# MisEty/GPS-SLAM

Measured on AMD Instinct MI355X. Metric: SLAM frames/sec @640x480, ~200k Gaussians; render PSNR vs ref, higher is better.
Workload: dtype f32; 1 GPU; synthetic RGB-D SLAM frames, independent scene per GPU; env_overrides=, full=False, schedule=overlap, windows=1, local_opt_interval=10, local_opt_iters=20, use_gt_pose=False, prologue_frames=25

## Files before the change

### gps_slam_amd/_lib.py

```python
import ctypes as C
import os

_HERE = os.path.dirname(os.path.abspath(__file__))
_LIBPATH = os.path.join(_HERE, "libgpsslam_hip.so")
_lib = None

vp, i32, i64, f32, f64 = C.c_void_p, C.c_int, C.c_int64, C.c_float, C.c_double


class TsdfState(C.Structure):
    _fields_ = [("width", i32), ("height", i32), ("fx", f32), ("fy", f32), ("cx", f32), ("cy", f32),
                ("voxel_size", f32), ("mu", f32), ("view_frustum_min", f32), ("view_frustum_max", f32),
                ("max_w", i32), ("n_blocks", i32), ("n_buckets", i32), ("n_excess", i32),
                ("vba", vp), ("vba_alloc_list", vp), ("hash", vp), ("excess_list", vp), ("counters", vp),
                ("alloc_prio", vp), ("scan_scratch", vp), ("visible_type", vp), ("visible_ids", vp), ("depth", vp),
                ("rgb", vp), ("minmax", vp), ("raycast", vp), ("icp_points", vp), ("icp_normals", vp),
                ("fv_visible_ids", vp), ("fv_minmax", vp), ("fv_raycast", vp), ("fv_colour", vp)]


class TsdfView(C.Structure):
    _fields_ = [("M", f32 * 16), ("invM", f32 * 16), ("fx", f32), ("fy", f32), ("cx", f32), ("cy", f32),
                ("visible_ids", vp), ("minmax", vp), ("raycast", vp), ("colour", vp), ("scratch", vp), ("counters", vp),
                ("w2c", f32 * 16), ("color_map", vp), ("vertex_map", vp), ("confidence_map", vp), ("depth_map", vp),
                ("depth_map_clamped", vp)]
# ... 52 lines not shown
    "gps_ssim_bwd": (i32, [i32, i32, i32, i32, i32, vp, vp, vp, vp, vp, vp, vp, vp]),
    "gps_upload_floats": (i32, [vp, vp, i32, vp]),
    "gps_isect_tiles": (i32, [i32, vp, vp, vp, i32, i32, i32, i64, vp, vp, vp, vp, vp, vp, i64, vp]),
    "gps_raster_raw_fwd": (i32, [i32, vp, vp, vp, vp, vp, i32, i32, i32, vp, vp, vp, vp, vp, vp, vp]),
    "gps_raster_raw_bwd": (i32, [i32, vp, vp, vp, vp, vp, i32, i32, i32, vp, vp, vp, vp, vp, vp, vp, vp, vp, vp, vp, vp,
                                 vp]),
    "gps_raster_ges_fwd": (i32, [i32, vp, vp, vp, vp, vp, i32, i32, i32, vp, vp, vp, f32, vp, vp, vp, vp]),
    "gps_raster_ges_bwd_gs": (i32, [i32, vp, vp, vp, vp, vp, vp, i32, i32, vp, vp, vp, f32, vp, vp, vp, vp, vp, vp,
                                    i32, vp]),
    "gps_raster_ges_bwd_strips": (i32, [i32, vp, vp, vp, vp, i32, vp, vp, i32, i32, vp, vp]),
    "gps_set_frame_chain_reserve": (None, [i32]),
    "gps_set_raster_fwd_persistent": (None, [i32]),

    "gps_raster_pack_records": (i32, [i32, vp, vp, vp, vp, vp, vp, vp]),
    "gps_raster_pair_image": (i32, [i32, i32, vp, vp, f32, vp, vp]),
    "gps_raster_ges_bwd_exact": (i32, [i32, vp, vp, vp, vp, vp, i32, i32, i32, vp, vp, vp, f32, vp, vp, vp, vp, vp, vp, vp]),
    "gps_compose_l1": (i32, [i32, i32, vp, vp, vp, vp, vp, vp, vp, vp, vp, vp, vp]),
    "gps_adam_step": (i32, [C.POINTER(AdamSegment), i32, f64, f64, f64, i32, vp]),
    "gps_loss_terms_workspace_floats": (i64, [i32, i32]),
    "gps_loss_terms": (i32, [i32, i32, vp, vp, vp, vp, vp, f32, vp, vp, f32, f32, vp, vp, vp, vp, vp, vp, vp, vp, vp]),
    "gps_loss_terms_exposure_partials": (i64, [i32, i32]),
    "gps_loss_terms_exposure": (i32, [i32, i32, vp, vp, vp, vp, vp, f32, vp, vp, f32, f32, vp, vp, vp, vp, vp, vp, vp, vp, vp, vp,
                                      vp]),
    "gps_exposure_slab_floats": (i64, [i32, i32]),
    "gps_compose_exposure": (i32, [i32, i32, vp, vp, vp, vp, vp, vp, vp, vp]),
    "gps_exposure_fwd": (i32, [i32, vp, vp, vp, vp]),
    "gps_exposure_bwd": (i32, [i32, vp, vp, vp, vp, vp, vp]),
    "gps_exposure_reduce": (i32, [vp, i32, i32, i32, vp, vp]),
    "gps_gauss_preprocess_fwd": (i32, [i32, i32, i32, vp, vp, vp, vp, vp, vp, vp, vp, vp, i32, i32, f32, f32, f32, f32,
                                       i32, vp, vp, vp, vp, vp, vp, vp, vp]),
    "gps_raster_ges_fwd_rec": (i32, [i32, vp, vp, i32, i32, vp, vp, vp, f32, vp, vp, vp]),
    "gps_raster_ges_fwd_rec_ordered": (i32, [i32, vp, vp, i32, i32, vp, vp, vp, f32, vp, vp, vp, vp]),
    "gps_isect_workspace_tile_order": (vp, [vp, i32, i64]),
    "gps_gauss_preprocess_bwd": (i32, [i32, i32, i32, vp, vp, vp, vp, vp, vp, vp, vp, vp, i32, i32, f32, vp, vp, vp, vp,
                                       vp, vp, vp, vp, vp, vp, vp, vp, vp]),
    "gps_gauss_preprocess_bwd_adam": (i32, [i32, i32, i32, vp, vp, vp, vp, vp, vp, vp, vp, vp, i32, i32, f32, vp, vp, vp,
                                            vp, vp, vp, vp, vp, vp, vp, vp, vp, vp, vp, f64, vp, f64, f64, f64, i32, vp]),
    "gps_tsdf_scratch_bytes": (i64, [i32, i32, i32, i32]),
    "gps_tsdf_reset": (i32, [C.POINTER(TsdfState), vp]),
    "gps_tsdf_rebuild_index": (i32, [C.POINTER(TsdfState), vp]),
    "gps_tsdf_mesh_workspace_bytes": (i64, [C.POINTER(TsdfState)]),
    "gps_tsdf_mesh_scene": (i32, [C.POINTER(TsdfState), i64, vp, vp, vp, i64, vp]),
    "gps_track_config_init": (i32, [C.POINTER(TrackConfig), C.c_char_p, i32, i32, f32, f32, f32, f32, i32, i32]),
    "gps_track_state_reset": (i32, [C.POINTER(TrackState)]),
    "gps_track_arg_line_alloc": (i32, [C.POINTER(vp)]),
    "gps_track_arg_line_free": (i32, [vp]),
    "gps_track_scratch_bytes": (i64, [i32, i32]),
    "gps_track_poll_profile": (i32, [vp, i32, i32, vp, vp]),
    "gps_track_poll_phases": (i32, [vp, i32, i32, vp, vp]),
    "gps_tsdf_track_camera": (i32, [C.POINTER(TsdfState), C.POINTER(TrackConfig), C.POINTER(TrackState), vp, i64, vp]),
    "gps_tsdf_process_frame_tracked": (i32, [C.POINTER(TsdfState), vp, C.POINTER(TrackConfig), C.POINTER(TrackState), vp, i64,
                                             vp]),
    "gps_tsdf_process_frame_tracked_gated": (i32, [C.POINTER(TsdfState), vp, C.POINTER(TrackConfig), C.POINTER(TrackState), vp, i64,
                                                   vp, vp, vp]),
    "gps_tsdf_convert_depth": (i32, [C.POINTER(TsdfState), vp, vp]),
    "gps_tsdf_allocate": (i32, [C.POINTER(TsdfState), vp, vp, vp]),
    "gps_tsdf_integrate": (i32, [C.POINTER(TsdfState), vp, vp]),
    "gps_tsdf_expected_depths": (i32, [C.POINTER(TsdfState), vp, i32, vp]),
    "gps_tsdf_expected_depths_partial": (i32, [C.POINTER(TsdfState), vp, i32, vp]),
    "gps_tsdf_raycast": (i32, [C.POINTER(TsdfState), vp, i32, i32, vp]),
    "gps_tsdf_expected_depths_and_raycast": (i32, [C.POINTER(TsdfState), vp, vp, i32, i32, vp]),
    "gps_tsdf_icp_maps": (i32, [C.POINTER(TsdfState), vp, vp]),
    "gps_tsdf_ray_stats": (i32, [C.POINTER(TsdfState), vp]),
    "gps_tsdf_ray_wave_rows": (i32, [C.POINTER(TsdfState), vp, i32, vp]),
    "gps_tsdf_find_visible": (i32, [C.POINTER(TsdfState), vp, vp]),
    "gps_tsdf_render_colour": (i32, [C.POINTER(TsdfState), vp]),
# ... 71 lines not shown
```

### gps_slam_amd/csrc/splat_bin.hpp

```cpp
#pragma once
#include "common.hpp"

namespace gps {

constexpr int BIN_BLOCK = 256;

struct TileBox { uint32_t x0, y0, x1, y1; };

__device__ __forceinline__ TileBox tile_bbox(float mx, float my, int radius_i, int tile_size, int tw, int th) {
    float radius = (float)radius_i;
    float ts = (float)tile_size;
    float tr = radius / ts, tx = mx / ts, ty = my / ts;
    TileBox b;
    float fx0 = floorf(tx - tr), fy0 = floorf(ty - tr), fx1 = ceilf(tx + tr), fy1 = ceilf(ty + tr);
    b.x0 = (uint32_t)fminf(fmaxf(fx0, 0.f), (float)tw);
    b.y0 = (uint32_t)fminf(fmaxf(fy0, 0.f), (float)th);
    b.x1 = (uint32_t)fminf(fmaxf(fx1, 0.f), (float)tw);
    b.y1 = (uint32_t)fminf(fmaxf(fy1, 0.f), (float)th);
    return b;
}

__device__ __forceinline__ void tile_group_count(float mx, float my, int r, int tile_size, int tw, int th, int& tiles, int& groups) {
    TileBox b = tile_bbox(mx, my, r, tile_size, tw, th);
    tiles = (int)((b.y1 - b.y0) * (b.x1 - b.x0));
    float rf = (float)r;
    groups = (int)((4 * rf * rf + 32 - 1) / 32);
}

constexpr int SB_MAX = 512;
constexpr int SB_MAX_TILES = 4096;
constexpr int BWD_CLASSES = GPS_BWD_CLASSES;
constexpr int BWD_BANDS = 16;
constexpr int BWD_KEYS = BWD_CLASSES * BWD_BANDS;
struct SbTables {
    uint32_t* C;
    uint32_t* P;
    uint32_t* tile_total;
    int32_t* cls_count;
    int32_t* cls_prefix;
    int sb_shift;
    int32_t* tile_order;
};
bool map_runs_beside_frame_chain();
int frame_chain_reserve_bits();
bool sb_supported(int N, int tile_width, int tile_height);
int sb_tables_clear(const struct SbTables& t, gps_stream stream);
__host__ __device__ inline int sb_shift_for(int N) {
    int s = 0;
    while ((((int64_t)N + 255) / 256 + ((int64_t)1 << s) - 1) >> s > SB_MAX) s++;
    return s;
}
__host__ __device__ inline int bwd_class(int r) { return r <= 4 ? 0 : r <= 8 ? 1 : r <= 16 ? 2 : r <= 32 ? 3 : 4; }
__host__ __device__ inline int bwd_key(int r, int n_tiles, unsigned y0, int th) {
    const int band = n_tiles > 0 ? (int)(y0 * (unsigned)BWD_BANDS / (unsigned)(th > 0 ? th : 1)) : 0;
    return bwd_class(r) * BWD_BANDS + (band < BWD_BANDS ? band : BWD_BANDS - 1);
}

struct BinCountOut {
    int32_t *tiles_per_gauss, *groups_per_gauss, *blk_tiles, *blk_groups, *blk_vis;
    int tile_size, tw, th;
    SbTables sb;
};

__device__ __forceinline__ void bin_block_sums(const BinCountOut& o, int t, int g, int vis) {
    __shared__ int red[3][BIN_BLOCK / 64];
    int ts = wave_sum_i(t), gs = wave_sum_i(g), vs = wave_sum_i(vis);
    if ((threadIdx.x & 63) == 0) { red[0][threadIdx.x >> 6] = ts; red[1][threadIdx.x >> 6] = gs; red[2][threadIdx.x >> 6] = vs; }
    __syncthreads();
    if (threadIdx.x == 0) {
        int a = 0, b = 0, c = 0;
        for (int w = 0; w < BIN_BLOCK / 64; w++) { a += red[0][w]; b += red[1][w]; c += red[2][w]; }
        o.blk_tiles[blockIdx.x] = a; o.blk_groups[blockIdx.x] = b; o.blk_vis[blockIdx.x] = c;
    }
}
// ... 48 lines not shown
```

### gps_slam_amd/csrc/splat_bin_sb.hip

```cpp
#include <mutex>

#include "launch_timing.hpp"
#include "splat_bin.hpp"

namespace {

using gps::BIN_BLOCK;
using gps::SB_MAX;
using gps::SB_MAX_TILES;
using gps::SbTables;
using gps::TileBox;
using gps::tile_bbox;

constexpr int SCAT_THREADS = 512;
constexpr int SCAT_WAVES = SCAT_THREADS / 64;
constexpr int SCAT_ITEMS = 4;
constexpr int SCAT_CHUNK = SCAT_THREADS * SCAT_ITEMS;

__device__ __forceinline__ int wave_max_i(int v) {
#pragma unroll
    for (int o = 32; o > 0; o >>= 1) v = max(v, __shfl_xor(v, o, 64));
    return v;
}
__device__ __forceinline__ int wave_min_i(int v) {
#pragma unroll
    for (int o = 32; o > 0; o >>= 1) v = min(v, __shfl_xor(v, o, 64));
    return v;
}
__device__ __forceinline__ int wave_excl_scan_i(int v, int& total) {
    const int incl = wave_incl_scan_i(v);
    total = __shfl(incl, 63, 64);
    return incl - v;
}

__global__ __launch_bounds__(256) void sb_scan_kernel(int n_tiles, SbTables t, gps::LaunchStamp stamp) {
    gps::StampScope timed(stamp);
    const int lane = threadIdx.x & 63, wave = threadIdx.x >> 6;
    const int tile = blockIdx.x * 4 + wave;
    static_assert(SB_MAX == 512, "a lane owns 8 consecutive superblocks");
    if (tile < n_tiles) {
        uint4* crow = reinterpret_cast<uint4*>(t.C + (size_t)tile * SB_MAX) + 2 * lane;
        const uint4 a = crow[0], b = crow[1];
        crow[0] = make_uint4(0, 0, 0, 0); crow[1] = make_uint4(0, 0, 0, 0);
        const int s = (int)(a.x + a.y + a.z + a.w + b.x + b.y + b.z + b.w);
        int total;
        uint32_t run = (uint32_t)wave_excl_scan_i(s, total);
        uint4 pa, pb;
        pa.x = run; run += a.x; pa.y = run; run += a.y; pa.z = run; run += a.z; pa.w = run; run += a.w;
        pb.x = run; run += b.x; pb.y = run; run += b.y; pb.z = run; run += b.z; pb.w = run;
        uint4* prow = reinterpret_cast<uint4*>(t.P + (size_t)tile * SB_MAX) + 2 * lane;
        prow[0] = pa; prow[1] = pb;
        if (lane == 0) t.tile_total[tile] = (uint32_t)total;
    }
    const int k = tile - n_tiles;
    if (k >= 0 && k < gps::BWD_KEYS) {
        int4* crow = reinterpret_cast<int4*>(t.cls_count + (size_t)k * SB_MAX) + 2 * lane;
        const int4 a = crow[0], b = crow[1];
        crow[0] = make_int4(0, 0, 0, 0); crow[1] = make_int4(0, 0, 0, 0);
        const int s = a.x + a.y + a.z + a.w + b.x + b.y + b.z + b.w;
        int total;
        int run = wave_excl_scan_i(s, total);
        int4 pa, pb;
        pa.x = run; run += a.x; pa.y = run; run += a.y; pa.z = run; run += a.z; pa.w = run; run += a.w;
        pb.x = run; run += b.x; pb.y = run; run += b.y; pb.z = run; run += b.z; pb.w = run;
        int4* prow = reinterpret_cast<int4*>(t.cls_prefix + (size_t)k * SB_MAX) + 2 * lane;
        prow[0] = pa; prow[1] = pb;
        if (lane == 0) t.cls_prefix[gps::BWD_KEYS * SB_MAX + k] = total;
    }
}

__global__ __launch_bounds__(SCAT_THREADS) void sb_scatter_kernel(
    int N, const float* __restrict__ means2d, const int32_t* __restrict__ radii, const int32_t* __restrict__ tiles_per_gauss,
    int tile_size, int tw, int th, SbTables t, int64_t isect_cap, int32_t* __restrict__ flatten_ids,
    int32_t* __restrict__ tile_offsets, int64_t* __restrict__ counts, int32_t* __restrict__ cls_ids,
    int32_t* __restrict__ cls_counts, int64_t cls_stride, gps::LaunchStamp stamp) {
    gps::StampScope timed(stamp);
    extern __shared__ uint32_t lds[];
    const int n_tiles = tw * th;
    if (blockIdx.x == gridDim.x - 1) {
        __shared__ int hist[64];
        __shared__ int gws[SCAT_WAVES];
        const int tid_ = threadIdx.x, lane_ = tid_ & 63, wave_ = tid_ >> 6;
        if (tid_ < 64) hist[tid_] = 0;
        const int per = (n_tiles + SCAT_THREADS - 1) / SCAT_THREADS;
        const int lo = min(n_tiles, tid_ * per), hi = min(n_tiles, lo + per);
        int sum = 0;
        for (int b = lo; b < hi; b++) sum += (int)t.tile_total[b];
        const int incl = wave_incl_scan_i(sum);
        if (lane_ == 63) gws[wave_] = incl;
        __syncthreads();
        int woff = 0, total = 0;
        for (int w = 0; w < SCAT_WAVES; w++) { const int v = gws[w]; if (w < wave_) woff += v; total += v; }
        int64_t run = woff + incl - sum;
        for (int b = lo; b < hi; b++) {
            const int tt = (int)t.tile_total[b];
            tile_offsets[b] = (int)min(run, isect_cap);
            atomicAdd(&hist[63 - min(63, tt >> 5)], 1);
            run += tt;
        }
        if (tid_ == 0) {
            int64_t ni = total;
            if (ni > isect_cap) { ni = isect_cap; counts[2] = 1; }
            counts[0] = ni; counts[1] = 0;
            int nv = 0;
            for (int k = 0; k < gps::BWD_CLASSES; k++) {
                int nk = 0;
                for (int b = 0; b < gps::BWD_BANDS; b++) nk += t.cls_prefix[gps::BWD_KEYS * SB_MAX + k * gps::BWD_BANDS + b];
                if (cls_counts) cls_counts[k] = nk;
                nv += nk;
            }
            counts[3] = nv;
        }
        __syncthreads();
        if (tid_ < 64) {
            int tot_;
            const int ex = wave_excl_scan_i(hist[tid_], tot_);
            hist[tid_] = ex;
        }
        __syncthreads();
        for (int b = tid_; b < n_tiles; b += SCAT_THREADS) t.tile_order[atomicAdd(&hist[63 - min(63, (int)(t.tile_total[b] >> 5))], 1)] = b;
        return;
    }
    const int sb = blockIdx.x, sb_size = BIN_BLOCK << t.sb_shift;
    uint32_t* base = lds;
    uint16_t* wavecnt = reinterpret_cast<uint16_t*>(lds + n_tiles);
    uint16_t* tot16 = wavecnt + SCAT_WAVES * n_tiles;
    uint32_t* pre = lds + n_tiles + ((SCAT_WAVES + 1) * n_tiles + 1) / 2;
    uint32_t* box = pre + sb_size + 1;
    __shared__ int ws[SCAT_WAVES], wlo[SCAT_WAVES], whi[SCAT_WAVES];
    __shared__ int key_wave[SCAT_WAVES][gps::BWD_KEYS];
    __shared__ int key_run[gps::BWD_KEYS];
    const int tid = threadIdx.x, lane = tid & 63, wave = tid >> 6;
    const int g0 = sb * sb_size;

    if (cls_ids && tid < gps::BWD_KEYS) {
        int start = t.cls_prefix[tid * SB_MAX + sb];
        for (int k = tid - tid % gps::BWD_BANDS; k < tid; k++) start += t.cls_prefix[gps::BWD_KEYS * SB_MAX + k];
        key_run[tid] = start;
        for (int w = 0; w < SCAT_WAVES; w++) key_wave[w][tid] = 0;
    }
    int carry = 0, row_lo = th, row_hi = 0;
    for (int j0 = 0; j0 < sb_size; j0 += SCAT_THREADS) {
        const int j = j0 + tid, g = g0 + j;
        const bool mine_j = j < sb_size;
        int tcount = 0, r = 0;
        uint32_t bx = 0;
        if (mine_j && g < N) {
            tcount = tiles_per_gauss[g];
            r = radii[g];
            if (tcount > 0) {
                const float2 m = *reinterpret_cast<const float2*>(means2d + 2 * (size_t)g);
                const TileBox b = tile_bbox(m.x, m.y, r, tile_size, tw, th);
                bx = b.x0 | (b.y0 << 12) | ((b.x1 - b.x0) << 24);
                row_lo = min(row_lo, (int)b.y0); row_hi = max(row_hi, (int)b.y1);
            }
// ... 12 lines not shown
        }
        __syncthreads();
        int woff = 0, total = 0;
        for (int w = 0; w < SCAT_WAVES; w++) { const int v = ws[w]; if (w < wave) woff += v; total += v; }
        if (mine_j) { pre[j] = (uint32_t)(carry + woff + incl - tcount); box[j] = bx; }
        carry += total;
        if (cls_ids) {
            if (key >= 0) {
                int before = 0;
                for (int w = 0; w < wave; w++) before += key_wave[w][key];
                cls_ids[(key / gps::BWD_BANDS) * cls_stride + key_run[key] + before + rank] = g;
            }
            __syncthreads();
            if (tid < gps::BWD_KEYS) {
                int all = 0;
                for (int w = 0; w < SCAT_WAVES; w++) { all += key_wave[w][tid]; key_wave[w][tid] = 0; }
                key_run[tid] += all;
            }
        }
    }
    const int n_pairs = carry;
    row_lo = wave_min_i(row_lo); row_hi = wave_max_i(row_hi);
    __syncthreads();
    if (lane == 0) { wlo[wave] = row_lo; whi[wave] = row_hi; }
    if (tid == 0) pre[sb_size] = (uint32_t)carry;
    __syncthreads();
    for (int w = 0; w < SCAT_WAVES; w++) { row_lo = min(row_lo, wlo[w]); row_hi = max(row_hi, whi[w]); }
    int t_lo = min(row_lo, row_hi) * tw, t_hi = row_hi * tw;
    if (t_hi < t_lo) t_hi = t_lo;
    const int nt = t_hi - t_lo;
    if (n_pairs == 0) return;

    {
        int before = 0;
        for (int b = tid; b < t_lo; b += SCAT_THREADS) before += (int)t.tile_total[b];
        const int per = (nt + SCAT_THREADS - 1) / SCAT_THREADS;
        const int lo = min(nt, tid * per), hi = min(nt, lo + per);
        int sum = 0;
        for (int b = lo; b < hi; b++) sum += (int)t.tile_total[t_lo + b];
        const int incl = wave_incl_scan_i(sum);
        before = wave_sum_i(before);
        __syncthreads();
        if (lane == 63) ws[wave] = incl;
        if (lane == 0) wlo[wave] = before;
        __syncthreads();
        int woff = 0, total = 0, front = 0;
        for (int w = 0; w < SCAT_WAVES; w++) { const int v = ws[w]; if (w < wave) woff += v; total += v; front += wlo[w]; }
        int run = front + woff + incl - sum;
        for (int b = lo; b < hi; b++) {
            base[b] = (uint32_t)run + t.P[(size_t)(t_lo + b) * SB_MAX + sb];
            run += (int)t.tile_total[t_lo + b];
        }
        (void)total;
    }
    int bits = 1;
    while ((1 << bits) < max(nt, 2)) bits++;
    const unsigned long long lt = lanemask_lt();
    uint16_t* mycnt = wavecnt + wave * n_tiles;
    for (int c0 = 0; c0 < n_pairs; c0 += SCAT_CHUNK) {
        for (int k = tid; k < nt; k += SCAT_THREADS) {
#pragma unroll
            for (int w = 0; w < SCAT_WAVES; w++) wavecnt[w * n_tiles + k] = 0;
        }
        __syncthreads();
        uint32_t tile[SCAT_ITEMS], gid[SCAT_ITEMS], rank[SCAT_ITEMS];
#pragma unroll
        for (int k = 0; k < SCAT_ITEMS; k++) {
            const int p = c0 + wave * (64 * SCAT_ITEMS) + k * 64 + lane;
            const bool valid = p < n_pairs;
            uint32_t d = 0;
            gid[k] = 0;
            if (valid) {
                int lo = 0, hi = sb_size;
                while (hi - lo > 1) { const int mid = (lo + hi) >> 1; if ((int)pre[mid] <= p) lo = mid; else hi = mid; }
                const uint32_t b = box[lo];
                const uint32_t w = b >> 24, q = (uint32_t)(p - (int)pre[lo]);
                d = ((b >> 12) & 0xfffu) * (uint32_t)tw + (b & 0xfffu) + (q / w) * (uint32_t)tw + q % w - (uint32_t)t_lo;
                gid[k] = (uint32_t)(g0 + lo);
            }
            tile[k] = d;
            unsigned long long same = __ballot(valid);
            for (int bb = 0; bb < bits; bb++) {
                const unsigned long long bal = __ballot(valid && ((d >> bb) & 1u));
                same &= ((d >> bb) & 1u) ? bal : ~bal;
            }
            const uint32_t prev = mycnt[d];
// ... 49 lines not shown
    static size_t granted[MAX_DEVICES] = {0};
    int dev = 0;
    if (hipGetDevice(&dev) != hipSuccess || dev < 0 || dev >= MAX_DEVICES) { (void)hipGetLastError(); return false; }
    std::lock_guard<std::mutex> lock(mu);
    if (lds <= granted[dev]) return true;
    if (hipFuncSetAttribute(reinterpret_cast<const void*>(sb_scatter_kernel), hipFuncAttributeMaxDynamicSharedMemorySize, (int)lds) != hipSuccess) {
        (void)hipGetLastError();
        return false;
    }
    granted[dev] = lds;
    return true;
}

size_t sb_tables_bytes() {
    return (size_t)SB_MAX_TILES * SB_MAX * 4 * 2 + (size_t)SB_MAX_TILES * 4 * 2 + (size_t)(SB_MAX + 1) * BWD_KEYS * 4 * 2 + 2048;
}

int sb_tables_clear(const SbTables& t, gps_stream stream) {
    hipStream_t s = (hipStream_t)stream;
    const bool ok = hipMemsetAsync(t.C, 0, (size_t)SB_MAX_TILES * SB_MAX * 4, s) == hipSuccess &&
                    hipMemsetAsync(t.cls_count, 0, (size_t)(SB_MAX + 1) * BWD_KEYS * 4, s) == hipSuccess;
    return ok ? GPS_OK : GPS_ERR_LAUNCH;
}

void sb_tables_carve(char* base, SbTables* t) {
    size_t off = 0;
    auto take = [&](size_t bytes) { char* p = base + off; off += (bytes + 255) & ~(size_t)255; return p; };
    t->C = (uint32_t*)take((size_t)SB_MAX_TILES * SB_MAX * 4);
    t->P = (uint32_t*)take((size_t)SB_MAX_TILES * SB_MAX * 4);
    t->tile_total = (uint32_t*)take((size_t)SB_MAX_TILES * 4);
    t->cls_count = (int32_t*)take((size_t)(SB_MAX + 1) * BWD_KEYS * 4);
    t->cls_prefix = (int32_t*)take((size_t)(SB_MAX + 1) * BWD_KEYS * 4);
    t->tile_order = (int32_t*)take((size_t)SB_MAX_TILES * 4);
    t->sb_shift = 0;
}

int isect_tiles_superblock(int N, const float* means2d, const int32_t* radii, const BinCountOut& cnt, int64_t isect_capacity,
                           const int32_t* tiles_per_gauss, int32_t* flatten_ids, int32_t* tile_offsets, int64_t* counts,
                           int32_t* cls_ids, int32_t* cls_counts, int64_t cls_stride, gps_stream stream) {
    GPS_ENTER();
    const int n_tiles = cnt.tw * cnt.th;
    hipStream_t s = (hipStream_t)stream;
    const bool ok = N > 0 && cnt.sb.C && isect_capacity > 0 && means2d && radii && tiles_per_gauss && flatten_ids && tile_offsets &&
                    counts && (!cls_ids || (cls_counts && cls_stride >= N)) && cnt.sb.sb_shift == sb_shift_for(N) &&
                    sb_supported(N, cnt.tw, cnt.th);
    if (!ok) {
        if (cnt.sb.C) (void)sb_tables_clear(cnt.sb, stream);
        return GPS_ERR_ARG;
    }
    const int nblk = gps_div_up(N, BIN_BLOCK);
    const int n_sb = (nblk + (1 << cnt.sb.sb_shift) - 1) >> cnt.sb.sb_shift;
    launch_kernel(TK_SB_SCAN, 0, sb_scan_kernel, dim3(gps_div_up(n_tiles + BWD_KEYS, 4)), dim3(256), 0, s, n_tiles, cnt.sb);
    const size_t lds = sb_scatter_lds_bytes(N, n_tiles);
    launch_kernel(TK_SB_SCATTER, 0, sb_scatter_kernel, dim3(n_sb + 1), dim3(SCAT_THREADS), lds, s, N, means2d, radii, tiles_per_gauss,
                  cnt.tile_size, cnt.tw, cnt.th, cnt.sb, isect_capacity, flatten_ids, tile_offsets, counts, cls_ids, cls_counts, cls_stride);
    GPS_LAUNCH_CHECK();
    return GPS_OK;
}

}
```

### gps_slam_amd/gsplat_ops.py

```python
import ctypes as C

import torch

from ._lib import AdamSegment, check, lib


def _ptr(t):
    return None if t is None else C.c_void_p(t.data_ptr())


def _stream():
    return C.c_void_p(torch.cuda.current_stream().cuda_stream)


def _f32c(t):
    assert t.is_cuda and t.dtype == torch.float32, "expects float32 GPU tensors"
    return t.contiguous()


def fully_fused_projection_fwd(means, quats, scales, viewmats, Ks, width, height, eps2d=0.3, near_plane=0.01,
                               far_plane=1e10, radius_clip=0.0):
    means, quats, scales = _f32c(means), _f32c(quats), _f32c(scales)
    viewmats, Ks = _f32c(viewmats), _f32c(Ks)
    assert viewmats.shape[0] == 1 and Ks.shape[0] == 1, "single camera (C == 1) as in raw_gs_model.cpp"
# ... 80 lines not shown
        N_ = radii.numel()
        icap, gcap = max(1 << 20, 16 * N_), max(1 << 20, 32 * N_)
        while True:
            r = isect_tiles_no_depth(means2d, radii, tile_size, tile_width, tile_height, icap, gcap, want_isect_ids)
            if int(r.counts[2]) == 0:
                return r
            icap, gcap = 2 * icap, 2 * gcap
    means2d = _f32c(means2d)
    radii = radii.contiguous()
    assert radii.dtype == torch.int32
    N = radii.numel()
    dev = means2d.device
    icap = int(isect_capacity or max(1 << 20, 16 * N))
    gcap = int(group_capacity or max(1 << 20, 32 * N))
    r = out if out is not None else IsectResult()
    if out is None:
        r.tiles_per_gauss = torch.empty((1, N), dtype=torch.int32, device=dev)
        r.isect_ids = torch.empty(icap, dtype=torch.int64, device=dev) if want_isect_ids else None
        r.flatten_ids = torch.empty(icap, dtype=torch.int32, device=dev)
        r.group_gs_ids = torch.empty(gcap, dtype=torch.int32, device=dev)
        r.group_starts = torch.empty(gcap, dtype=torch.int32, device=dev)
        r.isect_offsets = torch.empty((1, tile_height, tile_width), dtype=torch.int32, device=dev)
        r.counts = torch.zeros(4, dtype=torch.int64, device=dev)
        r.tile_width, r.tile_height = tile_width, tile_height
    nbytes = lib.gps_isect_workspace_bytes(N, icap)
    ws = _workspace(dev, nbytes)
    check(lib.gps_isect_tiles_no_depth(N, _ptr(means2d), _ptr(radii), tile_size, tile_width, tile_height, icap, gcap,
                                       _ptr(r.tiles_per_gauss), _ptr(r.isect_ids), _ptr(r.flatten_ids),
                                       _ptr(r.group_gs_ids), _ptr(r.group_starts), _ptr(r.isect_offsets),
                                       _ptr(r.counts), _ptr(ws), ws.numel(), _stream()), "gps_isect_tiles_no_depth")
    return r


def isect_tiles(means2d, radii, depths, tile_size, tile_width, tile_height, isect_capacity=None, want_isect_ids=True):
    if isect_capacity is None:
        icap = max(1 << 20, 16 * radii.numel())
        while True:
            r = isect_tiles(means2d, radii, depths, tile_size, tile_width, tile_height, icap, want_isect_ids)
            if int(r.counts[2]) == 0:
                return r
            icap *= 2
    means2d, depths = _f32c(means2d), _f32c(depths)
    radii = radii.contiguous()
    assert radii.dtype == torch.int32
    N = radii.numel()
    dev = means2d.device
    icap = int(isect_capacity or max(1 << 20, 16 * N))
    r = IsectResult()
    r.tiles_per_gauss = torch.empty((1, N), dtype=torch.int32, device=dev)
    r.isect_ids = torch.empty(icap, dtype=torch.int64, device=dev) if want_isect_ids else None
    r.flatten_ids = torch.empty(icap, dtype=torch.int32, device=dev)
    r.group_gs_ids = r.group_starts = None
    r.isect_offsets = torch.empty((1, tile_height, tile_width), dtype=torch.int32, device=dev)
    r.counts = torch.zeros(4, dtype=torch.int64, device=dev)
    r.tile_width, r.tile_height = tile_width, tile_height
    ws = _workspace(dev, lib.gps_isect_workspace_bytes(N, icap))
    check(lib.gps_isect_tiles(N, _ptr(means2d), _ptr(radii), _ptr(depths), tile_size, tile_width, tile_height, icap,
                              _ptr(r.tiles_per_gauss), _ptr(r.isect_ids), _ptr(r.flatten_ids), _ptr(r.isect_offsets),
                              _ptr(r.counts), _ptr(ws), ws.numel(), _stream()), "gps_isect_tiles")
    return r


def rasterize_to_pixels_fwd_ges(means2d, conics, colors, opacities, ref_depth_map, width, height, tile_size,
                                isect, delta_depth, want_last_ids=False):
    means2d, conics, colors, opacities = _f32c(means2d), _f32c(conics), _f32c(colors), _f32c(opacities)
    ref_depth_map = _f32c(ref_depth_map)
# ... 215 lines not shown
```

### include/gps_slam_hip.h

```cpp
#ifndef GPS_SLAM_HIP_H
#define GPS_SLAM_HIP_H

#include <stdint.h>

#ifdef __cplusplus
extern "C" {
#endif

typedef enum {
    GPS_OK = 0,
    GPS_ERR_ARG = -1,
    GPS_ERR_LAUNCH = -2,
    GPS_ERR_CAPACITY = -3
} gps_status;

typedef void *gps_stream;

#define GPS_API __attribute__((visibility("default")))

GPS_API const char *gps_version(void);
GPS_API const char *gps_build_flags(void);

#define GPS_TIMED_PREPROCESS_BWD 0
#define GPS_TIMED_PREPROCESS_FWD 1
// ... 23 lines not shown


GPS_API int gps_sh_fwd(int N, int K, int degrees_to_use, const float *dirs, const float *coeffs, const uint8_t *masks,
               float *colors, gps_stream stream);

GPS_API int gps_sh_bwd(int N, int K, int degrees_to_use, const float *dirs, const float *coeffs, const uint8_t *masks,
               const float *v_colors, float *v_coeffs, float *v_dirs, gps_stream stream);


GPS_API int64_t gps_isect_workspace_bytes(int N, int64_t isect_capacity);
GPS_API int gps_isect_workspace_init(void *workspace, int64_t workspace_bytes, gps_stream stream);

GPS_API int gps_isect_tiles_no_depth(int N, const float *means2d, const int32_t *radii, int tile_size, int tile_width,
                             int tile_height, int64_t isect_capacity, int64_t group_capacity,
                             int32_t *tiles_per_gauss, int64_t *isect_ids, int32_t *flatten_ids,
                             int32_t *group_gs_ids, int32_t *group_starts, int32_t *tile_offsets, int64_t *counts,
                             void *workspace, int64_t workspace_bytes, gps_stream stream);


GPS_API int gps_raster_ges_fwd(int N, const float *means2d, const float *conics, const float *colors,
                       const float *opacities, const float *ref_depth_map, int width, int height, int tile_size,
                       const int32_t *tile_offsets, const int32_t *flatten_ids, const int64_t *counts,
                       float delta_depth, float *render_colors, float *render_alphas, int32_t *last_ids,
                       gps_stream stream);

GPS_API int gps_raster_ges_fwd_rec(int N, const float *records, const float *ref_depth_map, int width, int height,
                                   const int32_t *tile_offsets, const int32_t *flatten_ids, const int64_t *counts,
                                   float delta_depth, float *render_colors, float *render_alphas, gps_stream stream);
GPS_API int gps_raster_ges_fwd_rec_ordered(int N, const float *records, const float *ref_depth_map, int width, int height,
                                           const int32_t *tile_offsets, const int32_t *flatten_ids, const int64_t *counts,
                                           float delta_depth, float *render_colors, float *render_alphas,
                                           const int32_t *tile_order, gps_stream stream);
GPS_API const int32_t *gps_isect_workspace_tile_order(void *workspace, int N, int64_t isect_capacity);

GPS_API int gps_raster_ges_bwd_gs(int N, const float *means2d, const float *conics, const float *colors,
                          const float *opacities, const int32_t *radii, const float *ref_depth_map, int width,
                          int height, const int32_t *group_gs_ids, const int32_t *group_starts,
                          const int64_t *counts, float delta_depth, const float *v_render_colors,
                          const float *v_render_alphas, float *v_means2d, float *v_conics, float *v_colors,
                          float *v_opacities, int accumulate, gps_stream stream);

#define GPS_BWD_CLASSES 5
GPS_API int gps_raster_ges_bwd_strips(int N, const float *records, const int32_t *radii, const int32_t *cls_ids,
                                      const int32_t *cls_counts, int cls_stride, const float *v_render_colors,
                                      const float *pix2, int width, int height, float *v_rows, gps_stream stream);
GPS_API void gps_set_frame_chain_reserve(int on);
GPS_API void gps_set_raster_fwd_persistent(int on);
GPS_API int gps_raster_pack_records(int N, const float *means2d, const float *conics, const float *colors,
                                    const float *opacities, const int32_t *radii, float *records, gps_stream stream);
GPS_API int gps_raster_pair_image(int width, int height, const float *v_render_alphas, const float *ref_depth_map,
                                  float delta_depth, float *pix2, gps_stream stream);

GPS_API int gps_raster_ges_bwd_exact(int N, const float *means2d, const float *conics, const float *colors,
                                     const float *opacities, const float *ref_depth_map, int width, int height,
                                     int tile_size, const int32_t *tile_offsets, const int32_t *flatten_ids,
                                     const int64_t *counts, float delta_depth, const float *v_render_colors,
                                     const float *v_render_alphas, float *v_means2d, float *v_conics, float *v_colors,
                                     float *v_opacities, gps_stream stream);


GPS_API int gps_ssim_fwd(int B, int CH, int H, int W, int channels_last, float C1, float C2, const float *img1,
                         const float *img2, float *ssim_map, float *dm_dmu1, float *dm_dsigma1_sq, float *dm_dsigma12,
                         gps_stream stream);

GPS_API int gps_ssim_bwd(int B, int CH, int H, int W, int channels_last, const float *img1, const float *img2,
                         const float *dL_dmap, const float *dm_dmu1, const float *dm_dsigma1_sq, const float *dm_dsigma12,
// ... 357 lines not shown
```

Baseline: 906.8 frames/s.

## Transpose superblock prefix table and move global tile offsets into scan kernel

The superblock scan kernel now handles 32 tiles per block and transposes the per-tile prefix table through LDS, so P is stored superblock-major. The scatter kernel can then read its row contiguously and add a precomputed global tile offset, instead of redoing a prefix over tile_total in every block. A last-block ticket in the scan kernel computes tile offsets, counts, class counts and the tile order, which removes the extra final scatter block. A standalone histogram kernel and a Python/C entry point for the superblock isect path are also added. The cost is a grid-wide atomic ticket plus threadfences, and the final work runs on one serial block.

```diff
diff --git a/gps_slam_amd/_lib.py b/gps_slam_amd/_lib.py
--- a/gps_slam_amd/_lib.py
+++ b/gps_slam_amd/_lib.py
@@ -108,6 +108,7 @@
     "gps_raster_ges_fwd_rec": (i32, [i32, vp, vp, i32, i32, vp, vp, vp, f32, vp, vp, vp]),
     "gps_raster_ges_fwd_rec_ordered": (i32, [i32, vp, vp, i32, i32, vp, vp, vp, f32, vp, vp, vp, vp]),
     "gps_isect_workspace_tile_order": (vp, [vp, i32, i64]),
+    "gps_isect_tiles_superblock": (i32, [i32, vp, vp, i32, i32, i32, i64, vp, vp, vp, vp, vp, vp, i64, vp, i64, vp]),
     "gps_gauss_preprocess_bwd": (i32, [i32, i32, i32, vp, vp, vp, vp, vp, vp, vp, vp, vp, i32, i32, f32, vp, vp, vp, vp,
                                        vp, vp, vp, vp, vp, vp, vp, vp, vp]),
     "gps_gauss_preprocess_bwd_adam": (i32, [i32, i32, i32, vp, vp, vp, vp, vp, vp, vp, vp, vp, i32, i32, f32, vp, vp, vp,
diff --git a/gps_slam_amd/csrc/splat_bin.hpp b/gps_slam_amd/csrc/splat_bin.hpp
--- a/gps_slam_amd/csrc/splat_bin.hpp
+++ b/gps_slam_amd/csrc/splat_bin.hpp
@@ -40,6 +40,7 @@
     int32_t* cls_prefix;
     int sb_shift;
     int32_t* tile_order;
+    uint32_t* ticket;
 };
 bool map_runs_beside_frame_chain();
 int frame_chain_reserve_bits();
diff --git a/gps_slam_amd/csrc/splat_bin_sb.hip b/gps_slam_amd/csrc/splat_bin_sb.hip
--- a/gps_slam_amd/csrc/splat_bin_sb.hip
+++ b/gps_slam_amd/csrc/splat_bin_sb.hip
@@ -33,94 +33,157 @@
     return incl - v;
 }
 
-__global__ __launch_bounds__(256) void sb_scan_kernel(int n_tiles, SbTables t, gps::LaunchStamp stamp) {
+constexpr int SCAN_THREADS = 512;
+constexpr int SCAN_WAVES = SCAN_THREADS / 64;
+constexpr int SCAN_TILES = 32;
+constexpr int SCAN_PER = SB_MAX_TILES / SCAN_THREADS;
+
+__device__ __forceinline__ uint32_t load_device(const uint32_t* p) { return __hip_atomic_load(p, __ATOMIC_RELAXED, __HIP_MEMORY_SCOPE_AGENT); }
+__device__ __forceinline__ int load_device(const int32_t* p) { return __hip_atomic_load(p, __ATOMIC_RELAXED, __HIP_MEMORY_SCOPE_AGENT); }
+
+__global__ __launch_bounds__(SCAN_THREADS) void sb_scan_kernel(int n_tiles, int n_sb, SbTables t, int64_t isect_cap,
+                                                               int32_t* __restrict__ tile_offsets, int64_t* __restrict__ counts,
+                                                               int32_t* __restrict__ cls_counts, gps::LaunchStamp stamp) {
     gps::StampScope timed(stamp);
-    const int lane = threadIdx.x & 63, wave = threadIdx.x >> 6;
-    const int tile = blockIdx.x * 4 + wave;
+    extern __shared__ uint32_t lds[];
+    const int tid = threadIdx.x, lane = tid & 63, wave = tid >> 6;
+    const int S = (n_sb + 63) & ~63;
+    const int n_groups = (n_tiles + SCAN_TILES - 1) / SCAN_TILES;
     static_assert(SB_MAX == 512, "a lane owns 8 consecutive superblocks");
-    if (tile < n_tiles) {
-        uint4* crow = reinterpret_cast<uint4*>(t.C + (size_t)tile * SB_MAX) + 2 * lane;
-        const uint4 a = crow[0], b = crow[1];
-        crow[0] = make_uint4(0, 0, 0, 0); crow[1] = make_uint4(0, 0, 0, 0);
-        const int s = (int)(a.x + a.y + a.z + a.w + b.x + b.y + b.z + b.w);
-        int total;
-        uint32_t run = (uint32_t)wave_excl_scan_i(s, total);
-        uint4 pa, pb;
-        pa.x = run; run += a.x; pa.y = run; run += a.y; pa.z = run; run += a.z; pa.w = run; run += a.w;
-        pb.x = run; run += b.x; pb.y = run; run += b.y; pb.z = run; run += b.z; pb.w = run;
-        uint4* prow = reinterpret_cast<uint4*>(t.P + (size_t)tile * SB_MAX) + 2 * lane;
-        prow[0] = pa; prow[1] = pb;
-        if (lane == 0) t.tile_total[tile] = (uint32_t)total;
-    }
-    const int k = tile - n_tiles;
-    if (k >= 0 && k < gps::BWD_KEYS) {
-        int4* crow = reinterpret_cast<int4*>(t.cls_count + (size_t)k * SB_MAX) + 2 * lane;
-        const int4 a = crow[0], b = crow[1];
-        crow[0] = make_int4(0, 0, 0, 0); crow[1] = make_int4(0, 0, 0, 0);
-        const int s = a.x + a.y + a.z + a.w + b.x + b.y + b.z + b.w;
-        int total;
-        int run = wave_excl_scan_i(s, total);
-        int4 pa, pb;
-        pa.x = run; run += a.x; pa.y = run; run += a.y; pa.z = run; run += a.z; pa.w = run; run += a.w;
-        pb.x = run; run += b.x; pb.y = run; run += b.y; pb.z = run; run += b.z; pb.w = run;
-        int4* prow = reinterpret_cast<int4*>(t.cls_prefix + (size_t)k * SB_MAX) + 2 * lane;
-        prow[0] = pa; prow[1] = pb;
-        if (lane == 0) t.cls_prefix[gps::BWD_KEYS * SB_MAX + k] = total;
-    }
+    static_assert(SCAN_TILES % SCAN_WAVES == 0 && SCAN_TILES == 32, "a wave takes SCAN_TILES / SCAN_WAVES rows; 32 tiles are one line of P");
+    if ((int)blockIdx.x < n_groups) {
+        constexpr int ROWS = SCAN_TILES / SCAN_WAVES;
+        const int t0 = blockIdx.x * SCAN_TILES;
+        const bool cols = 8 * lane < S;
+        uint4 a[ROWS], b[ROWS];
+#pragma unroll
+        for (int r = 0; r < ROWS; r++) {
+            const int tile = t0 + wave * ROWS + r;
+            a[r] = make_uint4(0, 0, 0, 0); b[r] = a[r];
+            if (tile < n_tiles && cols) {
+                uint4* crow = reinterpret_cast<uint4*>(t.C + (size_t)tile * SB_MAX) + 2 * lane;
+                a[r] = crow[0]; b[r] = crow[1];
+                crow[0] = make_uint4(0, 0, 0, 0); crow[1] = make_uint4(0, 0, 0, 0);
+            }
+        }
+#pragma unroll
+        for (int r = 0; r < ROWS; r++) {
+            const int tl = wave * ROWS + r, tile = t0 + tl;
+            const uint4 x = a[r], y = b[r];
+            const int s = (int)(x.x + x.y + x.z + x.w + y.x + y.y + y.z + y.w);
+            int total;
+            uint32_t run = (uint32_t)wave_excl_scan_i(s, total);
+            uint4 pa, pb;
+            pa.x = run; run += x.x; pa.y = run; run += x.y; pa.z = run; run += x.z; pa.w = run; run += x.w;
+            pb.x = run; run += y.x; pb.y = run; run += y.y; pb.z = run; run += y.z; pb.w = run;
+            if (cols) {
+                uint4* lrow = reinterpret_cast<uint4*>(lds) + tl * (S >> 2);
+                lrow[(2 * lane) ^ (tl & 15)] = pa; lrow[(2 * lane + 1) ^ (tl & 15)] = pb;
+            }
+            if (lane == 0 && tile < n_tiles) t.tile_total[tile] = (uint32_t)total;
+        }
+        __syncthreads();
+        const size_t stride = (size_t)n_groups * SCAN_TILES;
+        const int tq = tid & 7;
+        for (int sb = tid >> 3; sb < n_sb; sb += SCAN_THREADS / 8) {
+            uint32_t v[4];
+#pragma unroll
+            for (int i = 0; i < 4; i++) {
+                const int tl = 4 * tq + i;
+                v[i] = lds[tl * S + ((((sb >> 2) ^ (tl & 15)) << 2) | (sb & 3))];
+            }
+            *reinterpret_cast<uint4*>(t.P + (size_t)sb * stride + t0 + 4 * tq) = make_uint4(v[0], v[1], v[2], v[3]);
+        }
+    } else {
+        const int k = ((int)blockIdx.x - n_groups) * SCAN_WAVES + wave;
+        if (k < gps::BWD_KEYS) {
+            int4* crow = reinterpret_cast<int4*>(t.cls_count + (size_t)k * SB_MAX) + 2 * lane;
+            const int4 a = crow[0], b = crow[1];
+            crow[0] = make_int4(0, 0, 0, 0); crow[1] = make_int4(0, 0, 0, 0);
+            const int s = a.x + a.y + a.z + a.w + b.x + b.y + b.z + b.w;
+            int total;
+            int run = wave_excl_scan_i(s, total);
+            int4 pa, pb;
+            pa.x = run; run += a.x; pa.y = run; run += a.y; pa.z = run; run += a.z; pa.w = run; run += a.w;
+            pb.x = run; run += b.x; pb.y = run; run += b.y; pb.z = run; run += b.z; pb.w = run;
+            int4* prow = reinterpret_cast<int4*>(t.cls_prefix + (size_t)k * SB_MAX) + 2 * lane;
+            prow[0] = pa; prow[1] = pb;
+            if (lane == 0) t.cls_prefix[gps::BWD_KEYS * SB_MAX + k] = total;
+        }
+    }
+
+    int* hist = reinterpret_cast<int*>(lds);
+    int* gws = hist + 64;
+    int* knum = gws + SCAN_WAVES;
+    int* last = knum + gps::BWD_CLASSES;
+    __threadfence();
+    __syncthreads();
+    if (tid == 0) *last = atomicAdd(t.ticket, 1u) == gridDim.x - 1 ? 1 : 0;
+    __syncthreads();
+    if (!*last) return;
+    __threadfence();
+    if (tid == 0) *t.ticket = 0;
+    if (tid < 64) hist[tid] = 0;
+    const int per = (n_tiles + SCAN_THREADS - 1) / SCAN_THREADS;
+    const int lo = min(n_tiles, tid * per);
+    int tt[SCAN_PER];
+    int sum = 0;
+#pragma unroll
+    for (int i = 0; i < SCAN_PER; i++) {
+        tt[i] = i < per && lo + i < n_tiles ? (int)load_device(t.tile_total + lo + i) : 0;
+        sum += tt[i];
+    }
+    const int incl = wave_incl_scan_i(sum);
+    if (lane == 63) gws[wave] = incl;
+    static_assert(64 % gps::BWD_BANDS == 0, "the bands of a class sit in one wave");
+    if (tid < gps::BWD_KEYS) {
+        int v = load_device(t.cls_prefix + gps::BWD_KEYS * SB_MAX + tid);
+#pragma unroll
+        for (int o = gps::BWD_BANDS / 2; o > 0; o >>= 1) v += __shfl_xor(v, o, 64);
+        if (tid % gps::BWD_BANDS == 0) knum[tid / gps::BWD_BANDS] = v;
+    }
+    __syncthreads();
+    int woff = 0, total = 0;
+    for (int w = 0; w < SCAN_WAVES; w++) { const int v = gws[w]; if (w < wave) woff += v; total += v; }
+    int64_t run = woff + incl - sum;
+#pragma unroll
+    for (int i = 0; i < SCAN_PER; i++) {
+        if (i < per && lo + i < n_tiles) {
+            tile_offsets[lo + i] = (int)min(run, isect_cap);
+            atomicAdd(&hist[63 - min(63, tt[i] >> 5)], 1);
+            run += tt[i];
+        }
+    }
+    if (tid == 0) {
+        int64_t ni = total;
+        if (ni > isect_cap) { ni = isect_cap; counts[2] = 1; }
+        counts[0] = ni; counts[1] = 0;
+        int nv = 0;
+        for (int k = 0; k < gps::BWD_CLASSES; k++) {
+            if (cls_counts) cls_counts[k] = knum[k];
+            nv += knum[k];
+        }
+        counts[3] = nv;
+    }
+    __syncthreads();
+    if (tid < 64) {
+        int tot_;
+        const int ex = wave_excl_scan_i(hist[tid], tot_);
+        hist[tid] = ex;
+    }
+    __syncthreads();
+#pragma unroll
+    for (int i = 0; i < SCAN_PER; i++)
+        if (i < per && lo + i < n_tiles) t.tile_order[atomicAdd(&hist[63 - min(63, tt[i] >> 5)], 1)] = lo + i;
 }
 
 __global__ __launch_bounds__(SCAT_THREADS) void sb_scatter_kernel(
     int N, const float* __restrict__ means2d, const int32_t* __restrict__ radii, const int32_t* __restrict__ tiles_per_gauss,
     int tile_size, int tw, int th, SbTables t, int64_t isect_cap, int32_t* __restrict__ flatten_ids,
-    int32_t* __restrict__ tile_offsets, int64_t* __restrict__ counts, int32_t* __restrict__ cls_ids,
-    int32_t* __restrict__ cls_counts, int64_t cls_stride, gps::LaunchStamp stamp) {
+    const int32_t* __restrict__ tile_offsets, int32_t* __restrict__ cls_ids, int64_t cls_stride, gps::LaunchStamp stamp) {
     gps::StampScope timed(stamp);
     extern __shared__ uint32_t lds[];
     const int n_tiles = tw * th;
-    if (blockIdx.x == gridDim.x - 1) {
-        __shared__ int hist[64];
-        __shared__ int gws[SCAT_WAVES];
-        const int tid_ = threadIdx.x, lane_ = tid_ & 63, wave_ = tid_ >> 6;
-        if (tid_ < 64) hist[tid_] = 0;
-        const int per = (n_tiles + SCAT_THREADS - 1) / SCAT_THREADS;
-        const int lo = min(n_tiles, tid_ * per), hi = min(n_tiles, lo + per);
-        int sum = 0;
-        for (int b = lo; b < hi; b++) sum += (int)t.tile_total[b];
-        const int incl = wave_incl_scan_i(sum);
-        if (lane_ == 63) gws[wave_] = incl;
-        __syncthreads();
-        int woff = 0, total = 0;
-        for (int w = 0; w < SCAT_WAVES; w++) { const int v = gws[w]; if (w < wave_) woff += v; total += v; }
-        int64_t run = woff + incl - sum;
-        for (int b = lo; b < hi; b++) {
-            const int tt = (int)t.tile_total[b];
-            tile_offsets[b] = (int)min(run, isect_cap);
-            atomicAdd(&hist[63 - min(63, tt >> 5)], 1);
-            run += tt;
-        }
-        if (tid_ == 0) {
-            int64_t ni = total;
-            if (ni > isect_cap) { ni = isect_cap; counts[2] = 1; }
-            counts[0] = ni; counts[1] = 0;
-            int nv = 0;
-            for (int k = 0; k < gps::BWD_CLASSES; k++) {
-                int nk = 0;
-                for (int b = 0; b < gps::BWD_BANDS; b++) nk += t.cls_prefix[gps::BWD_KEYS * SB_MAX + k * gps::BWD_BANDS + b];
-                if (cls_counts) cls_counts[k] = nk;
-                nv += nk;
-            }
-            counts[3] = nv;
-        }
-        __syncthreads();
-        if (tid_ < 64) {
-            int tot_;
-            const int ex = wave_excl_scan_i(hist[tid_], tot_);
-            hist[tid_] = ex;
-        }
-        __syncthreads();
-        for (int b = tid_; b < n_tiles; b += SCAT_THREADS) t.tile_order[atomicAdd(&hist[63 - min(63, (int)(t.tile_total[b] >> 5))], 1)] = b;
-        return;
-    }
     const int sb = blockIdx.x, sb_size = BIN_BLOCK << t.sb_shift;
     uint32_t* base = lds;
     uint16_t* wavecnt = reinterpret_cast<uint16_t*>(lds + n_tiles);
@@ -199,26 +262,8 @@
     if (n_pairs == 0) return;
 
     {
-        int before = 0;
-        for (int b = tid; b < t_lo; b += SCAT_THREADS) before += (int)t.tile_total[b];
-        const int per = (nt + SCAT_THREADS - 1) / SCAT_THREADS;
-        const int lo = min(nt, tid * per), hi = min(nt, lo + per);
-        int sum = 0;
-        for (int b = lo; b < hi; b++) sum += (int)t.tile_total[t_lo + b];
-        const int incl = wave_incl_scan_i(sum);
-        before = wave_sum_i(before);
-        __syncthreads();
-        if (lane == 63) ws[wave] = incl;
-        if (lane == 0) wlo[wave] = before;
-        __syncthreads();
-        int woff = 0, total = 0, front = 0;
-        for (int w = 0; w < SCAT_WAVES; w++) { const int v = ws[w]; if (w < wave) woff += v; total += v; front += wlo[w]; }
-        int run = front + woff + incl - sum;
-        for (int b = lo; b < hi; b++) {
-            base[b] = (uint32_t)run + t.P[(size_t)(t_lo + b) * SB_MAX + sb];
-            run += (int)t.tile_total[t_lo + b];
-        }
-        (void)total;
+        const uint32_t* prow = t.P + (size_t)sb * (size_t)((n_tiles + 31) & ~31) + t_lo;
+        for (int b = tid; b < nt; b += SCAT_THREADS) base[b] = (uint32_t)tile_offsets[t_lo + b] + prow[b];
     }
     int bits = 1;
     while ((1 << bits) < max(nt, 2)) bits++;
@@ -334,6 +379,7 @@
     t->cls_count = (int32_t*)take((size_t)(SB_MAX + 1) * BWD_KEYS * 4);
     t->cls_prefix = (int32_t*)take((size_t)(SB_MAX + 1) * BWD_KEYS * 4);
     t->tile_order = (int32_t*)take((size_t)SB_MAX_TILES * 4);
+    t->ticket = (uint32_t*)take(4);
     t->sb_shift = 0;
 }
 
@@ -352,12 +398,71 @@
     }
     const int nblk = gps_div_up(N, BIN_BLOCK);
     const int n_sb = (nblk + (1 << cnt.sb.sb_shift) - 1) >> cnt.sb.sb_shift;
-    launch_kernel(TK_SB_SCAN, 0, sb_scan_kernel, dim3(gps_div_up(n_tiles + BWD_KEYS, 4)), dim3(256), 0, s, n_tiles, cnt.sb);
+    const int n_groups = gps_div_up(n_tiles, SCAN_TILES);
+    const size_t scan_lds = (size_t)SCAN_TILES * ((n_sb + 63) & ~63) * 4;
+    launch_kernel(TK_SB_SCAN, 0, sb_scan_kernel, dim3(n_groups + gps_div_up(BWD_KEYS, SCAN_WAVES)), dim3(SCAN_THREADS), scan_lds, s,
+                  n_tiles, n_sb, cnt.sb, isect_capacity, tile_offsets, counts, cls_counts);
     const size_t lds = sb_scatter_lds_bytes(N, n_tiles);
-    launch_kernel(TK_SB_SCATTER, 0, sb_scatter_kernel, dim3(n_sb + 1), dim3(SCAT_THREADS), lds, s, N, means2d, radii, tiles_per_gauss,
-                  cnt.tile_size, cnt.tw, cnt.th, cnt.sb, isect_capacity, flatten_ids, tile_offsets, counts, cls_ids, cls_counts, cls_stride);
+    launch_kernel(TK_SB_SCATTER, 0, sb_scatter_kernel, dim3(n_sb), dim3(SCAT_THREADS), lds, s, N, means2d, radii, tiles_per_gauss,
+                  cnt.tile_size, cnt.tw, cnt.th, cnt.sb, isect_capacity, flatten_ids, (const int32_t*)tile_offsets, cls_ids, cls_stride);
     GPS_LAUNCH_CHECK();
     return GPS_OK;
 }
 
 }
+
+namespace {
+
+__global__ __launch_bounds__(gps::BIN_BLOCK) void sb_histogram_kernel(int N, const float* __restrict__ means2d,
+                                                                      const int32_t* __restrict__ radii,
+                                                                      const int32_t* __restrict__ tiles_per_gauss, int tile_size,
+                                                                      int tw, int th, SbTables t) {
+    __shared__ uint32_t hist[SB_MAX_TILES];
+    __shared__ int khist[gps::BWD_KEYS];
+    const int nt = tw * th, g = blockIdx.x * BIN_BLOCK + threadIdx.x;
+    for (int b = threadIdx.x; b < nt; b += BIN_BLOCK) hist[b] = 0;
+    if (threadIdx.x < gps::BWD_KEYS) khist[threadIdx.x] = 0;
+    __syncthreads();
+    if (g < N && radii[g] > 0) {
+        const int r = radii[g], n = tiles_per_gauss[g];
+        unsigned y0 = 0;
+        if (n > 0) {
+            const TileBox tb = tile_bbox(means2d[2 * (size_t)g], means2d[2 * (size_t)g + 1], r, tile_size, tw, th);
+            y0 = tb.y0;
+            for (uint32_t ty = tb.y0; ty < tb.y1; ty++)
+                for (uint32_t tx = tb.x0; tx < tb.x1; tx++) atomicAdd(&hist[ty * (uint32_t)tw + tx], 1u);
+        }
+        atomicAdd(&khist[gps::bwd_key(r, n, y0, th)], 1);
+    }
+    __syncthreads();
+    const int sb = (int)blockIdx.x >> t.sb_shift;
+    for (int b = threadIdx.x; b < nt; b += BIN_BLOCK) {
+        const uint32_t c = hist[b];
+        if (c) atomicAdd(&t.C[(size_t)b * SB_MAX + sb], c);
+    }
+    if (threadIdx.x < gps::BWD_KEYS) {
+        const int c = khist[threadIdx.x];
+        if (c) atomicAdd(&t.cls_count[threadIdx.x * SB_MAX + sb], c);
+    }
+}
+
+}
+
+extern "C" int gps_isect_tiles_superblock(int N, const float* means2d, const int32_t* radii, int tile_size, int tile_width,
+                                          int tile_height, int64_t isect_capacity, int32_t* tiles_per_gauss, int32_t* flatten_ids,
+                                          int32_t* tile_offsets, int64_t* counts, int32_t* cls_ids, int32_t* cls_counts,
+                                          int64_t cls_stride, void* workspace, int64_t workspace_bytes, gps_stream stream) {
+    GPS_ENTER();
+    GPS_REQUIRE(N > 0 && tile_size > 0 && isect_capacity > 0 && isect_capacity < (1ll << 31) && means2d && radii && tiles_per_gauss &&
+                flatten_ids && tile_offsets && counts && (!cls_ids || (cls_counts && cls_stride >= N)));
+    GPS_REQUIRE(gps::sb_supported(N, tile_width, tile_height));
+    gps::BinCountOut cnt;
+    const int r = gps::isect_count_targets(N, isect_capacity, tiles_per_gauss, tile_size, tile_width, tile_height, workspace,
+                                           workspace_bytes, true, &cnt);
+    if (r != GPS_OK) return r;
+    sb_histogram_kernel<<<dim3(gps_div_up(N, BIN_BLOCK)), dim3(BIN_BLOCK), 0, (hipStream_t)stream>>>(
+        N, means2d, radii, tiles_per_gauss, tile_size, tile_width, tile_height, cnt.sb);
+    if (hipGetLastError() != hipSuccess) return GPS_ERR_LAUNCH;
+    return gps::isect_tiles_superblock(N, means2d, radii, cnt, isect_capacity, tiles_per_gauss, flatten_ids, tile_offsets, counts,
+                                       cls_ids, cls_counts, cls_stride, stream);
+}
diff --git a/gps_slam_amd/gsplat_ops.py b/gps_slam_amd/gsplat_ops.py
--- a/gps_slam_amd/gsplat_ops.py
+++ b/gps_slam_amd/gsplat_ops.py
@@ -136,6 +136,34 @@
     return r
 
 
+def isect_workspace(dev, N, isect_capacity):
+    ws = torch.empty(int(lib.gps_isect_workspace_bytes(N, int(isect_capacity))), dtype=torch.uint8, device=dev)
+    check(lib.gps_isect_workspace_init(_ptr(ws), ws.numel(), _stream()), "gps_isect_workspace_init")
+    return ws
+
+
+def isect_tiles_superblock(means2d, radii, tiles_per_gauss, tile_size, tile_width, tile_height, isect_capacity, workspace,
+                           want_classes=False, flatten_ids=None):
+    means2d, radii, tiles_per_gauss = _f32c(means2d), radii.contiguous(), tiles_per_gauss.contiguous()
+    assert radii.dtype == torch.int32 and tiles_per_gauss.dtype == torch.int32
+    N, dev, icap = radii.numel(), means2d.device, int(isect_capacity)
+    if flatten_ids is None:
+        flatten_ids = torch.empty(icap, dtype=torch.int32, device=dev)
+    assert flatten_ids.numel() >= icap
+    tile_offsets = torch.empty((tile_height, tile_width), dtype=torch.int32, device=dev)
+    counts = torch.zeros(4, dtype=torch.int64, device=dev)
+    cls_ids = torch.empty((5, N), dtype=torch.int32, device=dev) if want_classes else None
+    cls_counts = torch.empty(5, dtype=torch.int32, device=dev) if want_classes else None
+    check(lib.gps_isect_tiles_superblock(N, _ptr(means2d), _ptr(radii), tile_size, tile_width, tile_height, icap,
+                                         _ptr(tiles_per_gauss), _ptr(flatten_ids), _ptr(tile_offsets), _ptr(counts),
+                                         _ptr(cls_ids), _ptr(cls_counts), N, _ptr(workspace), workspace.numel(), _stream()),
+          "gps_isect_tiles_superblock")
+    order_ptr = lib.gps_isect_workspace_tile_order(_ptr(workspace), N, icap)
+    off = (order_ptr - workspace.data_ptr()) // 4
+    tile_order = workspace.view(torch.int32)[off:off + tile_width * tile_height]
+    return flatten_ids, tile_offsets, counts, cls_ids, cls_counts, tile_order
+
+
 def isect_tiles(means2d, radii, depths, tile_size, tile_width, tile_height, isect_capacity=None, want_isect_ids=True):
     if isect_capacity is None:
         icap = max(1 << 20, 16 * radii.numel())
diff --git a/include/gps_slam_hip.h b/include/gps_slam_hip.h
--- a/include/gps_slam_hip.h
+++ b/include/gps_slam_hip.h
@@ -79,6 +79,11 @@
                                            float delta_depth, float *render_colors, float *render_alphas,
                                            const int32_t *tile_order, gps_stream stream);
 GPS_API const int32_t *gps_isect_workspace_tile_order(void *workspace, int N, int64_t isect_capacity);
+
+GPS_API int gps_isect_tiles_superblock(int N, const float *means2d, const int32_t *radii, int tile_size, int tile_width,
+                                       int tile_height, int64_t isect_capacity, int32_t *tiles_per_gauss, int32_t *flatten_ids,
+                                       int32_t *tile_offsets, int64_t *counts, int32_t *cls_ids, int32_t *cls_counts,
+                                       int64_t cls_stride, void *workspace, int64_t workspace_bytes, gps_stream stream);
 
 GPS_API int gps_raster_ges_bwd_gs(int N, const float *means2d, const float *conics, const float *colors,
                           const float *opacities, const int32_t *radii, const float *ref_depth_map, int width,
```

Result: slower. 876.5 frames/s (-3.3%).
